# awslabs/dgl-ke

Hardware: NVIDIA H100
Metric: edges/sec TransE_l2 d=400 neg=200 at 1/2/4/8 H100 vs ref CPU; HBM GB/s %peak (higher is better)
Workload: dtype f32

## Files before the change

### dgl-ke_b200/csrc/kge_fused.cu

```cuda
#include <cuda.h>
#include <cstdio>
#include <cstdlib>
#include "kge_common.cuh"
#include "kge_tc.cuh"

namespace kge {

using namespace tc;

namespace {

constexpr int kTileM = 128;
constexpr int kThreadsF = 384;
constexpr int kProducerWarp = 8;
constexpr int kMaxS1 = 4, kMaxS2 = 8;
constexpr int kMaxPf = 8;
constexpr uint32_t kRingBytes = 192 * 1024;
constexpr int kWc = 128;
constexpr float kLog2e = 1.4426950408889634f;
constexpr float kLn2 = 0.6931471805599453f;

struct FusedArgs {
  int model, adversarial;
  float gamma, Tl2e, inv2B, uni;
  float reg_coef;
  int reg_norm;
  int C, Rx, Ry, D;
  int N1;
  int nblkD;
  int nS1, nS2;
  uint32_t stage1Bytes, stage2Bytes;
  float *VhiT, *VloT;
  float* colpart;
  int ncolpart;
  const float* x2;
  const float* y2;
  const float* pos;
  const float* wt;
  const float* wbar;
  float *gpos, *rowsum, *pl, *nl;
  float* dumpS;
// ... 53 lines not shown
  };
  for (long long k = 0; k < n && k < S; ++k) load(k);
  const int L = g.pf_lag < S - 1 ? g.pf_lag : (S > 2 ? S - 2 : 1);
  for (long long k = 0; k < n; ++k) {
    const int s = (int)(k % S);
    mbar_wait(&pf_full[w][s], (uint32_t)((k / S) & 1));
    const long long v = vrow(k);
    float* dst = v < nU ? g.pf_nc + v * (long long)g.D : g.pf_bn + (v - nU) * (long long)g.D;
    const long long kr = k - L + S;
    const bool reload = k >= L && kr < n;
    if (reload && kr >= base + 32) { base += 32; ids_lo = ids_hi; ids_hi = fetch_ids(base + 32); }
    if (elect_one()) {
      bulk_s2g(dst, slots + (size_t)s * g.pf_row_bytes, g.pf_row_bytes);
      bulk_commit();
      if (reload) { if (L == 3) bulk_wait_read<3>(); else if (L == 2) bulk_wait_read<2>(); else bulk_wait_read<1>(); }
    }
    __syncwarp();
    if (reload) load(kr);
  }
  if (elect_one()) bulk_wait_all();
  __syncwarp();
}

template <int NV>
__global__ void __launch_bounds__(kThreadsF, 1)
k_fused_pos(const __grid_constant__ CUtensorMap mXh, const __grid_constant__ CUtensorMap mXl,
            const __grid_constant__ CUtensorMap mYh1, const __grid_constant__ CUtensorMap mYl1,
            const __grid_constant__ CUtensorMap mYh2, const __grid_constant__ CUtensorMap mYl2, FusedArgs g) {
  extern __shared__ __align__(1024) uint8_t smem_raw[];
  __shared__ __align__(8) uint64_t full1[kMaxS1], empty1[kMaxS1], full2[kMaxS2], empty2[kMaxS2];
  __shared__ __align__(8) uint64_t pf_full[2][kMaxPf];
  __shared__ __align__(16) float colA[NV];
  __shared__ __align__(16) float cpart[8][NV];

  const int warp = threadIdx.x >> 5, lane = threadIdx.x & 31;
  uint8_t* ring = (uint8_t*)(((uintptr_t)smem_raw + 1023) & ~(uintptr_t)1023);

  const int mtiles = (g.Rx + kTileM - 1) / kTileM;
  const int ntiles = g.C * mtiles;
  const int nkb1 = (g.D + 31) >> 5;
  const int nkb2 = (g.Ry + 31) >> 5;
  const int nchunks = (g.D + kWc - 1) / kWc;
  constexpr uint32_t yBytes1 = (uint32_t)NV * 128u;
  constexpr uint32_t yBytes2 = (uint32_t)kWc * 128u;
  const bool l2 = g.model == KGE_TRANSE_L2;

  if (threadIdx.x == 0) {
    for (int s = 0; s < kMaxS1; ++s) { mbar_init(&full1[s], 1); mbar_init(&empty1[s], 8); }
    for (int s = 0; s < kMaxS2; ++s) { mbar_init(&full2[s], 1); mbar_init(&empty2[s], 8); }
    for (int s = 0; s < kMaxPf; ++s) { mbar_init(&pf_full[0][s], 1); mbar_init(&pf_full[1][s], 1); }
    asm volatile("fence.mbarrier_init.release.cluster;" ::: "memory");
  }
  if (warp == kProducerWarp && lane == 0) {
    tma_prefetch_desc(&mXh); tma_prefetch_desc(&mXl); tma_prefetch_desc(&mYh1);
    tma_prefetch_desc(&mYl1); tma_prefetch_desc(&mYh2); tma_prefetch_desc(&mYl2);
  }
  __syncthreads();

  if (warp >= 8) {
  asm volatile("setmaxnreg.dec.sync.aligned.u32 56;");
  if (warp == kProducerWarp) {
    uint32_t n1 = 0, n2 = 0;
    for (int tile = blockIdx.x; tile < ntiles; tile += gridDim.x) {
      const int c = tile / mtiles, m0 = (tile % mtiles) * kTileM;
      for (uint32_t k = (n2 > (uint32_t)g.nS2 ? n2 - g.nS2 : 0); k < n2; ++k) mbar_wait(&empty2[k % g.nS2], (k / g.nS2) & 1);
      for (int kb = 0; kb < nkb1; ++kb, ++n1) {
        const uint32_t s = n1 % g.nS1;
        mbar_wait(&empty1[s], ((n1 / g.nS1) & 1) ^ 1);
        uint8_t* st = ring + (size_t)s * g.stage1Bytes;
        const int yx = (c * g.nblkD + kb) * g.Rx + m0;
        const int yy = (c * g.nblkD + kb) * g.Ry;
        if (elect_one()) {
          mbar_expect_tx(&full1[s], 2u * 16384u + 2u * yBytes1);
          tma_load_2d(st, &mXh, &full1[s], 0, yx);
          tma_load_2d(st + 16384, &mXl, &full1[s], 0, yx);
          tma_load_2d(st + 32768, &mYh1, &full1[s], 0, yy);
          tma_load_2d(st + 32768 + yBytes1, &mYl1, &full1[s], 0, yy);
        }
        __syncwarp();
      }
      for (uint32_t k = (n1 > (uint32_t)g.nS1 ? n1 - g.nS1 : 0); k < n1; ++k) mbar_wait(&empty1[k % g.nS1], (k / g.nS1) & 1);
      for (int ch = 0; ch < nchunks; ++ch) {
        for (int kb = 0; kb < nkb2; ++kb, ++n2) {
          const uint32_t s = n2 % g.nS2;
          mbar_wait(&empty2[s], ((n2 / g.nS2) & 1) ^ 1);
          uint8_t* st = ring + (size_t)s * g.stage2Bytes;
          const int yy = (c * nkb2 + kb) * g.D + ch * kWc;
          if (elect_one()) {
            mbar_expect_tx(&full2[s], 2u * yBytes2);
            tma_load_2d(st, &mYh2, &full2[s], 0, yy);
            tma_load_2d(st + yBytes2, &mYl2, &full2[s], 0, yy);
          }
          __syncwarp();
        }
      }
    }
  } else if (warp >= 10 && g.pf_slots > 0) {
    prefetch_rows(g, ring, pf_full, warp - 10, lane);
  }
  } else {
    asm volatile("setmaxnreg.inc.sync.aligned.u32 224;");
    const int wg = warp >> 2, q = lane & 3;
    const int et = threadIdx.x;
    const int rloc = wg * 64 + (warp & 3) * 16 + (lane >> 2);
    uint32_t n1 = 0, n2 = 0;
    float acc[NV / 2];
    for (int tile = blockIdx.x; tile < ntiles; tile += gridDim.x) {
      const int c = tile / mtiles, m0 = (tile % mtiles) * kTileM;
      epi_bar();
      for (int y = et; y < NV; y += 256) {
        const bool ok = y < g.Ry;
        colA[y] = (l2 && ok) ? g.y2[(long long)c * g.Ry + y] : 0.f;
      }
      epi_bar();
#pragma unroll
      for (int i = 0; i < NV / 2; ++i) acc[i] = 0.f;
      for (int kb = 0; kb < nkb1; ++kb, ++n1) {
        const uint32_t s = n1 % g.nS1;
        mbar_wait(&full1[s], (n1 / g.nS1) & 1);
        const uint32_t st = smem_u32(ring + (size_t)s * g.stage1Bytes);
        const uint64_t dXh = make_desc(st + wg * 8192u), dXl = make_desc(st + 16384u + wg * 8192u);
        const uint64_t dYh = make_desc(st + 32768u), dYl = make_desc(st + 32768u + yBytes1);
        const int kleft = g.D - kb * 32;
        const int ksteps = kleft >= 32 ? 4 : (kleft >> 3);
        wgmma_fence();
        for (int ks = 0; ks < ksteps; ++ks) {
          const uint64_t o = (uint64_t)(ks * 2);
          wgmma_ss<NV>(acc, dXh + o, dYh + o, 1u);
          wgmma_ss<NV>(acc, dXh + o, dYl + o, 1u);
          wgmma_ss<NV>(acc, dXl + o, dYh + o, 1u);
        }
        wgmma_commit();
        if (kb > 0) {
          wgmma_wait<1>();
          if (lane == 0) mbar_arrive(&empty1[(n1 - 1) % g.nS1]);
        }
      }
      wgmma_wait<0>();
      if (lane == 0) mbar_arrive(&empty1[(n1 - 1) % g.nS1]);
      reg_fence(acc);

      float rscal[2];
#pragma unroll
      for (int h = 0; h < 2; ++h) {
        const int m = m0 + rloc + 8 * h;
        const bool row_ok = m < g.Rx;
        const long long gx = (long long)c * g.Rx + (row_ok ? m : 0);
        const float x2v = (l2 && row_ok) ? g.x2[gx] : 0.f;
        const float w_i = (g.wt && row_ok) ? g.wt[gx] : 1.f;
        const float kw = w_i * g.inv2B;
        float mxl = -INFINITY;
        if (g.adversarial || g.dumpS) {
#pragma unroll
          for (int j = 0; j < NV / 8; ++j) {
            float sv[2];
// ... 37 lines not shown
            const float u = 1.f + t;
            const float r1 = rcpa(u);
            const float sig = (s >= 0.f) ? r1 : t * r1;
            const float sp = fmaf(kLn2, lg2a(u), fmaxf(s, 0.f));
            const bool ok = row_ok && (col < g.Ry);
            const float coef = ok ? pe * sig * kw * rinv : 0.f;
            if (ok) { nls = fmaf(pe, sp, nls); den += pe; }
            rs += coef;
            acc[4 * j + 2 * h + e] = coef;
          }
        }
        den += __shfl_xor_sync(0xffffffffu, den, 1); den += __shfl_xor_sync(0xffffffffu, den, 2);
        nls += __shfl_xor_sync(0xffffffffu, nls, 1); nls += __shfl_xor_sync(0xffffffffu, nls, 2);
        rs += __shfl_xor_sync(0xffffffffu, rs, 1); rs += __shfl_xor_sync(0xffffffffu, rs, 2);
        const float rscale = g.adversarial ? (row_ok ? 1.f / den : 0.f) : g.uni;
        rscal[h] = rscale;
        if (g.dumpV && row_ok) {
#pragma unroll
          for (int j = 0; j < NV / 8; ++j)
            if (8 * j + 2 * q < g.Ry)
              *reinterpret_cast<float2*>(g.dumpV + gx * g.Ry + 8 * j + 2 * q) =
                  make_float2(acc[4 * j + 2 * h] * rscale, acc[4 * j + 2 * h + 1] * rscale);
        }
        {
          float* vh = g.VhiT + slabT_off(c, g.Rx, g.Ry, m, 0);
          float* vl = g.VloT + slabT_off(c, g.Rx, g.Ry, m, 0);
#pragma unroll
          for (int j = 0; j < NV / 8; ++j) {
#pragma unroll
            for (int e = 0; e < 2; ++e) {
              const int col = 8 * j + 2 * q + e;
              const float v = acc[4 * j + 2 * h + e] * rscale;
              if (row_ok && col < g.Ry) {
                float hi, lo;
                split_tf32(v, hi, lo);
                vh[col * 32] = hi; vl[col * 32] = lo;
              }
              if (l2) {
                float s = v;
                s += __shfl_xor_sync(0xffffffffu, s, 4);
                s += __shfl_xor_sync(0xffffffffu, s, 8);
                s += __shfl_xor_sync(0xffffffffu, s, 16);
                if (lane < 4) cpart[warp][col] = h ? cpart[warp][col] + s : s;
              }
            }
          }
        }
        if (q == 0 && row_ok) {
          const float ps = g.pos[gx];
          const float wb = g.wt ? *g.wbar : 1.f;
          g.pl[gx] = softplusf(-ps);
          g.nl[gx] = nls * rscale * w_i;
          g.gpos[gx] = -sigmoidf(-ps) * wb * g.inv2B;
          if (l2) g.rowsum[gx] = rs * rscale;
        }
      }
      if (l2) {
        epi_bar();
        float* dst = g.colpart + (long long)(tile % mtiles) * g.C * g.Ry + (long long)c * g.Ry;
        for (int y = et; y < g.Ry; y += 256) {
          float s = cpart[0][y];
#pragma unroll
          for (int w = 1; w < 8; ++w) s += cpart[w][y];
          dst[y] = s;
        }
      }
      {
        const int srcLo = (lane & ~3) | (q >> 1), srcHi = srcLo + 2;
        const bool odd = q & 1;
#pragma unroll
        for (int j = 0; j < NV / 8; ++j) {
          float o[4];
#pragma unroll
          for (int h = 0; h < 2; ++h) {
            const float v0 = acc[4 * j + 2 * h], v1 = acc[4 * j + 2 * h + 1];
            const float a0 = __shfl_sync(0xffffffffu, v0, srcLo), a1 = __shfl_sync(0xffffffffu, v1, srcLo);
            const float b0 = __shfl_sync(0xffffffffu, v0, srcHi), b1 = __shfl_sync(0xffffffffu, v1, srcHi);
            o[h] = odd ? a1 : a0;
            o[2 + h] = odd ? b1 : b0;
          }
          acc[4 * j + 0] = o[0]; acc[4 * j + 1] = o[1]; acc[4 * j + 2] = o[2]; acc[4 * j + 3] = o[3];
        }
      }

      for (int ch = 0; ch < nchunks; ++ch) {
        const int d0 = ch * kWc;
        float acc2[kWc / 2];
#pragma unroll
        for (int i = 0; i < kWc / 2; ++i) acc2[i] = 0.f;
#pragma unroll
        for (int kb = 0; kb < (NV + 31) / 32; ++kb) {
          if (kb >= nkb2) break;
          const uint32_t s = n2 % g.nS2;
          mbar_wait(&full2[s], (n2 / g.nS2) & 1);
          const uint32_t st = smem_u32(ring + (size_t)s * g.stage2Bytes);
          const uint64_t dYh = make_desc(st), dYl = make_desc(st + yBytes2);
          const int kleft = g.Ry - kb * 32;
          const int ksteps = kleft >= 32 ? 4 : (kleft >> 3);
          uint32_t ah[2][4] = {}, al[2][4] = {};
#pragma unroll
          for (int ks = 0; ks < 4; ++ks) {
            const int j = kb * 4 + ks;
            if (j < NV / 8 && ks < ksteps) {
              if (ks >= 2) wgmma_wait<1>();
#pragma unroll
              for (int r = 0; r < 4; ++r) {
                float hi, lo;
                split_tf32(acc[4 * j + r], hi, lo);
                ah[ks & 1][r] = __float_as_uint(hi); al[ks & 1][r] = __float_as_uint(lo);
              }
              wgmma_fence();
              const uint64_t o = (uint64_t)(ks * 2);
              wgmma_rs<kWc>(acc2, ah[ks & 1], dYh + o, 1u);
              wgmma_rs<kWc>(acc2, ah[ks & 1], dYl + o, 1u);
              wgmma_rs<kWc>(acc2, al[ks & 1], dYh + o, 1u);
              wgmma_commit();
              if (ks >= 1) { reg_fence(ah[(ks - 1) & 1]); reg_fence(al[(ks - 1) & 1]); }
            }
          }
          wgmma_wait<0>();
          reg_fence(ah[0]); reg_fence(ah[1]); reg_fence(al[0]); reg_fence(al[1]);
          if (lane == 0) mbar_arrive(&empty2[s]);
          ++n2;
        }
        reg_fence(acc2);
#pragma unroll
        for (int h = 0; h < 2; ++h) {
          const int m = m0 + rloc + 8 * h;
          if (m >= g.Rx) continue;
          float* orow = g.out + ((long long)c * g.Rx + m) * (long long)g.D;
#pragma unroll
          for (int j = 0; j < kWc / 8; ++j) {
            const int k = d0 + 8 * j + 2 * q;
            if (k >= g.D) continue;
            *reinterpret_cast<float2*>(orow + k) = make_float2(acc2[4 * j + 2 * h] * rscal[h], acc2[4 * j + 2 * h + 1] * rscal[h]);
          }
        }
      }
    }
  }
}

template <int NW, int KS>
__device__ __forceinline__ void neg_kblock(float (&acc)[NW / 2], uint64_t dVh, uint64_t dVl, uint64_t dAh, uint64_t dAl) {
  wgmma_fence();
#pragma unroll
  for (int ks = 0; ks < KS; ++ks) {
    const uint64_t o = (uint64_t)(ks * 2);
    wgmma_ss<NW>(acc, dVh + o, dAh + o, 1u);
    wgmma_ss<NW>(acc, dVh + o, dAl + o, 1u);
    wgmma_ss<NW>(acc, dVl + o, dAh + o, 1u);
  }
  wgmma_commit();
}

constexpr int kNegEpiLoads = 16;

template <int NW, bool FLAT>
__global__ void __launch_bounds__(kThreadsF, 1)
k_fused_neg(const __grid_constant__ CUtensorMap mVh, const __grid_constant__ CUtensorMap mVl,
            const __grid_constant__ CUtensorMap mAh, const __grid_constant__ CUtensorMap mAl, FusedArgs g) {
  extern __shared__ __align__(1024) uint8_t smem_raw[];
  __shared__ __align__(8) uint64_t full[kMaxS1], empty[kMaxS1];
  __shared__ __align__(8) uint64_t pf_full[2][kMaxPf];

  const int warp = threadIdx.x >> 5, lane = threadIdx.x & 31;
  uint8_t* ring = (uint8_t*)(((uintptr_t)smem_raw + 1023) & ~(uintptr_t)1023);

  const int mtiles = (g.Rx + kTileM - 1) / kTileM;
  const int ntiles = g.C * mtiles;
  const int nkb = (g.Ry + 31) >> 5;
  const int nch = (g.D + NW - 1) / NW;
  constexpr uint32_t aBytes = (uint32_t)kTileM * 128u;
  constexpr uint32_t bBytes = (uint32_t)NW * 128u;
  const bool l2 = g.model == KGE_TRANSE_L2;

  if (threadIdx.x == 0) {
// ... 84 lines not shown
          if (FLAT) {
            bh[jj] = __ldg(reinterpret_cast<const float2*>(brow[h] + k));
          } else {
            const long long so = boff[h] + (k >> 5) * blk + (k & 31);
            bh[jj] = __ldg(reinterpret_cast<const float2*>(g.Xhi + so));
            bl[jj] = __ldg(reinterpret_cast<const float2*>(g.Xlo + so));
          }
        }
      };
      float gsq[2] = {0.f, 0.f};
      for (int ch = 0; ch < nch; ++ch) {
        const int d0 = ch * NW;
        float acc[NW / 2];
#pragma unroll
        for (int i = 0; i < NW / 2; ++i) acc[i] = 0.f;
        for (int kb = 0; kb < nkb; ++kb, ++n) {
          const uint32_t s = n % g.nS1;
          mbar_wait(&full[s], (n / g.nS1) & 1);
          const uint32_t st = smem_u32(ring + (size_t)s * g.stage1Bytes);
          const uint64_t dVh = make_desc(st + wg * 8192u), dVl = make_desc(st + aBytes + wg * 8192u);
          const uint64_t dAh = make_desc(st + 2 * aBytes), dAl = make_desc(st + 2 * aBytes + bBytes);
          const int kleft = g.Ry - kb * 32;
          const int ksteps = kleft >= 32 ? 4 : (kleft >> 3);
          switch (ksteps) {
            case 4: neg_kblock<NW, 4>(acc, dVh, dVl, dAh, dAl); break;
            case 3: neg_kblock<NW, 3>(acc, dVh, dVl, dAh, dAl); break;
            case 2: neg_kblock<NW, 2>(acc, dVh, dVl, dAh, dAl); break;
            default: neg_kblock<NW, 1>(acc, dVh, dVl, dAh, dAl); break;
          }
          if (kb > 0) {
            wgmma_wait<1>();
            if (lane == 0) mbar_arrive(&empty[(n - 1) % g.nS1]);
          }
        }
        if (early) load_b(0, d0, 0);
        wgmma_wait<0>();
        if (lane == 0) mbar_arrive(&empty[(n - 1) % g.nS1]);
        reg_fence(acc);
#pragma unroll
        for (int h = 0; h < 2; ++h) {
          if (!rok[h]) continue;
          float* orow = g.out + ((long long)c * g.Rx + m0 + rloc + 8 * h) * (long long)g.D;
#pragma unroll
          for (int j0 = 0; j0 < NJ; j0 += NB) {
            if (!early || h > 0 || j0 > 0) load_b(h, d0, j0);
#pragma unroll
            for (int jj = 0; jj < NB; ++jj) {
              const int j = j0 + jj;
              const int k = d0 + 8 * j + 2 * q;
              if (j >= NJ || k >= g.D) continue;
              float o0 = acc[4 * j + 2 * h], o1 = acc[4 * j + 2 * h + 1];
              const float2 b = FLAT ? bh[jj] : make_float2(bh[jj].x + bl[jj].x, bh[jj].y + bl[jj].y);
// ... 5 lines not shown
            }
          }
        }
      }
#pragma unroll
      for (int h = 0; h < 2; ++h) {
        float v = gsq[h];
        v += __shfl_xor_sync(0xffffffffu, v, 1);
        v += __shfl_xor_sync(0xffffffffu, v, 2);
        const int m = m0 + rloc + 8 * h;
        if (q == 0 && m < g.Rx) g.gsn[(long long)c * g.Rx + m] = v / (float)g.D;
      }
    }
  }
}

}

bool fused_supported(const StepParams& p) {
  return umma_supported(p) && !p.hinge && !p.pairwise && !p.neg_deg && p.Cs <= 240 && p.Ns <= 240;
}

namespace {
struct Geometry { int Rx, Ry, N1, nS1, nS2, pf_slots; uint32_t stage1Bytes, stage2Bytes, pf_off; bool ok; };

int neg_chunk_width(int D, bool want_prefetch) {
  static const int widths[] = {64, 128, 200, 256};
  int best = 0;
  long long best_rows = 0;
  for (int w : widths) {
    if (w == 256 && want_prefetch) continue;
    const long long rows = (long long)((D + w - 1) / w) * (kTileM + w);
    if (!best || rows < best_rows) { best = w; best_rows = rows; }
  }
  return best;
}

Geometry geometry(const StepParams& p, int mode, bool want_prefetch) {
  Geometry q{};
  const uint32_t row = (uint32_t)p.D * 4u;
  if (mode == 1) {
    q.Rx = p.Ns; q.Ry = p.Cs;
    q.N1 = neg_chunk_width(p.D, want_prefetch);
    q.stage1Bytes = 2u * kTileM * 128u + 2u * (uint32_t)q.N1 * 128u;
    q.nS1 = (int)(kRingBytes / q.stage1Bytes); if (q.nS1 > kMaxS1) q.nS1 = kMaxS1;
    q.ok = q.nS1 >= 2;
    if (q.ok && want_prefetch) {
      int nS = q.nS1;
      while (nS > 2 && kRingBytes - (uint32_t)nS * q.stage1Bytes < 2u * kMaxPf * row) --nS;
      const uint32_t used = (uint32_t)nS * q.stage1Bytes;
      int slots = (int)((kRingBytes - used) / (2u * row));
      if (slots > kMaxPf) slots = kMaxPf;
      if (slots >= 2) { q.pf_slots = slots; q.nS1 = nS; q.pf_off = used; }
    }
    return q;
  }
  q.Rx = p.Cs; q.Ry = p.Ns;
  q.N1 = q.Ry <= 64 ? 64 : (q.Ry <= 128 ? 128 : (q.Ry <= 208 ? 208 : 256));
  q.stage1Bytes = 2u * 16384u + 2u * (uint32_t)q.N1 * 128u;
  q.stage2Bytes = 2u * (uint32_t)kWc * 128u;
  q.nS1 = (int)(kRingBytes / q.stage1Bytes); if (q.nS1 > kMaxS1) q.nS1 = kMaxS1;
  q.nS2 = (int)(kRingBytes / q.stage2Bytes); if (q.nS2 > kMaxS2) q.nS2 = kMaxS2;
  q.ok = q.nS1 >= 2 && q.nS2 >= 2;
  if (q.ok && want_prefetch) {
    int nS1 = q.nS1, nS2 = q.nS2;
    uint32_t want = 2u * kMaxPf * row;
    while (nS1 > 2 && kRingBytes - (uint32_t)nS1 * q.stage1Bytes < want) --nS1;
    uint32_t used = (uint32_t)nS1 * q.stage1Bytes;
    if (want > kRingBytes - used) want = kRingBytes - used;
    while (nS2 > 4 && kRingBytes - (uint32_t)nS2 * q.stage2Bytes < want) --nS2;
    if ((uint32_t)nS2 * q.stage2Bytes > used) used = (uint32_t)nS2 * q.stage2Bytes;
    int slots = (int)((kRingBytes - used) / (2u * row));
    if (slots > kMaxPf) slots = kMaxPf;
    if (slots >= 2) { q.pf_slots = slots; q.nS1 = nS1; q.nS2 = nS2; q.pf_off = used; }
  }
  return q;
}

int launch_error() {
  const cudaError_t e = cudaGetLastError();
  return e == cudaSuccess ? KGE_OK : fail(KGE_ERR_CUDA, "k_fused launch: %s", cudaGetErrorString(e));
}
template <int NV>
int launch_pos(const LaunchCtx& c, int grid, size_t smem, const CUtensorMap* m, const FusedArgs& g) {
  if (int rc = smem_optin((const void*)k_fused_pos<NV>, smem)) return rc;
  KGE_LAUNCH_NAMED(c, "k_fused<P: S=A.Bn^T, loss, GA=V.Bn>", (k_fused_pos<NV>), grid, kThreadsF, smem,
                   m[0], m[1], m[2], m[3], m[4], m[5], g);
  return launch_error();
}
template <int NW, bool FLAT>
int launch_neg_src(const LaunchCtx& c, int grid, size_t smem, const CUtensorMap* m, const FusedArgs& g) {
  if (int rc = smem_optin((const void*)k_fused_neg<NW, FLAT>, smem)) return rc;
  KGE_LAUNCH_NAMED(c, "k_fused<N: G_neg=V^T.A, mean sq>", (k_fused_neg<NW, FLAT>), grid, kThreadsF, smem, m[0], m[1], m[2], m[3], g);
  return launch_error();
}
template <int NW>
int launch_neg(const LaunchCtx& c, int grid, size_t smem, const CUtensorMap* m, const FusedArgs& g) {
  return (g.xraw || g.xids) ? launch_neg_src<NW, true>(c, grid, smem, m, g) : launch_neg_src<NW, false>(c, grid, smem, m, g);
}
int launch_width(const LaunchCtx& c, bool P, int grid, size_t smem, const CUtensorMap* m, const FusedArgs& g) {
  switch (g.N1) {
    case 64: return P ? launch_pos<64>(c, grid, smem, m, g) : launch_neg<64>(c, grid, smem, m, g);
    case 128: return P ? launch_pos<128>(c, grid, smem, m, g) : launch_neg<128>(c, grid, smem, m, g);
    case 200: return launch_neg<200>(c, grid, smem, m, g);
    case 208: return launch_pos<208>(c, grid, smem, m, g);
    default: return P ? launch_pos<256>(c, grid, smem, m, g) : launch_neg<256>(c, grid, smem, m, g);
  }
}
}

int fused_prefetch_slots(const StepParams& p, int mode) { return geometry(p, mode, true).pf_slots; }

int fused_launch(const LaunchCtx& c, const StepParams& p, const StepWs& w, int mode, const float* wt, float* dumpS,
                 float* dumpV, const TableView* ent, const long long* neg_ids, const FusedPrefetch* pf) {
  FusedArgs g{};
  g.model = p.model; g.adversarial = p.adversarial;
  g.gamma = p.gamma; g.Tl2e = p.adv_temperature * kLog2e; g.inv2B = 0.5f / (float)p.B; g.uni = 1.f / (float)p.Ns;
  g.reg_coef = p.reg_coef; g.reg_norm = p.reg_norm;
  g.C = p.C; g.D = p.D; g.nblkD = slab_blocks(p.D);
  const bool P = mode == 0;
  const Geometry q = geometry(p, mode, pf != nullptr && ent != nullptr);
  if (!q.ok) return fail(KGE_ERR_UNSUPPORTED, "fused kernel: shape does not fit (N1=%d)", q.N1);
  g.Rx = q.Rx; g.Ry = q.Ry; g.N1 = q.N1; g.nS1 = q.nS1; g.nS2 = q.nS2;
  g.stage1Bytes = q.stage1Bytes; g.stage2Bytes = q.stage2Bytes;
  if (pf && ent && q.pf_slots >= 2) {
    static const int lag_env = getenv("KGE_B200_PF_LAG") ? atoi(getenv("KGE_B200_PF_LAG")) : 1;
    g.pf_lag = lag_env < 1 ? 1 : (lag_env > 3 ? 3 : lag_env);
    g.pf_slots = q.pf_slots; g.pf_off = q.pf_off; g.pf_row_bytes = (uint32_t)p.D * 4u; g.pf_parity = mode;
    g.pf_node_ids = pf->node_ids; g.pf_nU_dev = pf->nU_dev; g.pf_nU = pf->nU; g.pf_nNeg = pf->nNeg;
    g.pf_neg_ids = pf->neg_ids; g.pf_nc = pf->nc; g.pf_bn = pf->bn;
    g.xtab = *ent;
  }
  g.VhiT = w.VhiT; g.VloT = w.VloT; g.colpart = w.colpart; g.ncolpart = (p.Cs + kTileM - 1) / kTileM;
  g.dumpV = dumpV;
  const size_t smem = kRingBytes + 1024;
  const int mtiles = (g.Rx + kTileM - 1) / kTileM;
  int grid = p.C * mtiles;
  if (grid > c.num_sms) grid = c.num_sms;
  CUtensorMap m[6];
  if (P) {
    g.x2 = w.a2; g.y2 = w.b2;
    g.pos = w.pos; g.wt = wt; g.wbar = w.wbar;
    g.gpos = w.gpos; g.rowsum = w.rowsum; g.pl = w.pl; g.nl = w.nl;
    g.dumpS = dumpS;
    g.out = w.GA;
    const long long rowsX = (long long)p.C * p.Cs * g.nblkD, rowsY = (long long)p.C * p.Ns * g.nblkD;
    const long long rowsYT = (long long)p.C * slab_blocks(p.Ns) * p.D;
    if (tc_make_map(&m[0], w.Ahi, rowsX, 32, kTileM) || tc_make_map(&m[1], w.Alo, rowsX, 32, kTileM) ||
        tc_make_map(&m[2], w.Bhi, rowsY, 32, g.N1) || tc_make_map(&m[3], w.Blo, rowsY, 32, g.N1) ||
        tc_make_map(&m[4], w.BhiT, rowsYT, 32, kWc) || tc_make_map(&m[5], w.BloT, rowsYT, 32, kWc))
      return KGE_ERR_CUDA;
    return launch_width(c, true, grid, smem, m, g);
  }
  g.Xhi = w.Bhi; g.Xlo = w.Blo;
  if (ent && ent->n_shards == 1 && neg_ids) { g.xids = neg_ids; g.xtab = *ent; }
  if (w.BnRaw) g.xraw = w.BnRaw;
  g.gsn = w.gsn;
  g.out = w.Bn;
  const long long rowsV = (long long)p.C * slab_blocks(p.Cs) * p.Ns, rowsA = (long long)p.C * slab_blocks(p.Cs) * p.D;
  if (tc_make_map(&m[0], w.VhiT, rowsV, 32, kTileM) || tc_make_map(&m[1], w.VloT, rowsV, 32, kTileM) ||
      tc_make_map(&m[2], w.AhiT, rowsA, 32, g.N1) || tc_make_map(&m[3], w.AloT, rowsA, 32, g.N1))
    return KGE_ERR_CUDA;
  return launch_width(c, false, grid, smem, m, g);
}

}
```

### dgl-ke_b200/csrc/kge_tc.cuh

```cuda
#pragma once
#include <cuda.h>
#include <cuda_runtime.h>
#include <stdint.h>

namespace kge {
namespace tc {

__device__ __forceinline__ uint32_t smem_u32(const void* p) { return (uint32_t)__cvta_generic_to_shared(p); }

__device__ __forceinline__ bool elect_one() {
  uint32_t pred = 0;
  asm volatile(
      "{\n\t.reg .pred P1;\n\t"
      "elect.sync _|P1, 0xFFFFFFFF;\n\t"
      "selp.b32 %0, 1, 0, P1;\n\t}"
      : "=r"(pred));
  return pred != 0;
}

__device__ __forceinline__ void mbar_init(uint64_t* bar, uint32_t count) {
  asm volatile("mbarrier.init.shared::cta.b64 [%0], %1;" ::"r"(smem_u32(bar)), "r"(count));
}
__device__ __forceinline__ void mbar_expect_tx(uint64_t* bar, uint32_t bytes) {
  asm volatile("mbarrier.arrive.expect_tx.shared::cta.b64 _, [%0], %1;" ::"r"(smem_u32(bar)), "r"(bytes) : "memory");
// ... 66 lines not shown
}
template <>
__device__ __forceinline__ void wgmma_ss<200>(float (&d)[100], uint64_t adesc, uint64_t bdesc, uint32_t accumulate) {
  asm volatile("{\n\t.reg .pred p;\n\tsetp.ne.b32 p, %102, 0;\n\t"
               "wgmma.mma_async.sync.aligned.m64n200k8.f32.tf32.tf32 {%0,%1,%2,%3,%4,%5,%6,%7,%8,%9,%10,%11,%12,%13,%14,%15,%16,%17,%18,%19,%20,%21,%22,%23,%24,%25,%26,%27,%28,%29,%30,%31,%32,%33,%34,%35,%36,%37,%38,%39,%40,%41,%42,%43,%44,%45,%46,%47,%48,%49,%50,%51,%52,%53,%54,%55,%56,%57,%58,%59,%60,%61,%62,%63,%64,%65,%66,%67,%68,%69,%70,%71,%72,%73,%74,%75,%76,%77,%78,%79,%80,%81,%82,%83,%84,%85,%86,%87,%88,%89,%90,%91,%92,%93,%94,%95,%96,%97,%98,%99}, %100, %101, p, 1, 1;\n\t}"
               : KGE_D32(0), KGE_D32(32), KGE_D32(64), KGE_D4(96)
               : "l"(adesc), "l"(bdesc), "r"(accumulate));
}
template <>
__device__ __forceinline__ void wgmma_ss<208>(float (&d)[104], uint64_t adesc, uint64_t bdesc, uint32_t accumulate) {
  asm volatile("{\n\t.reg .pred p;\n\tsetp.ne.b32 p, %106, 0;\n\t"
               "wgmma.mma_async.sync.aligned.m64n208k8.f32.tf32.tf32 {%0,%1,%2,%3,%4,%5,%6,%7,%8,%9,%10,%11,%12,%13,%14,%15,%16,%17,%18,%19,%20,%21,%22,%23,%24,%25,%26,%27,%28,%29,%30,%31,%32,%33,%34,%35,%36,%37,%38,%39,%40,%41,%42,%43,%44,%45,%46,%47,%48,%49,%50,%51,%52,%53,%54,%55,%56,%57,%58,%59,%60,%61,%62,%63,%64,%65,%66,%67,%68,%69,%70,%71,%72,%73,%74,%75,%76,%77,%78,%79,%80,%81,%82,%83,%84,%85,%86,%87,%88,%89,%90,%91,%92,%93,%94,%95,%96,%97,%98,%99,%100,%101,%102,%103}, %104, %105, p, 1, 1;\n\t}"
               : KGE_D32(0), KGE_D32(32), KGE_D32(64), KGE_D4(96), KGE_D4(100)
               : "l"(adesc), "l"(bdesc), "r"(accumulate));
}
template <>
__device__ __forceinline__ void wgmma_ss<256>(float (&d)[128], uint64_t adesc, uint64_t bdesc, uint32_t accumulate) {
  asm volatile("{\n\t.reg .pred p;\n\tsetp.ne.b32 p, %130, 0;\n\t"
               "wgmma.mma_async.sync.aligned.m64n256k8.f32.tf32.tf32 {%0,%1,%2,%3,%4,%5,%6,%7,%8,%9,%10,%11,%12,%13,%14,%15,%16,%17,%18,%19,%20,%21,%22,%23,%24,%25,%26,%27,%28,%29,%30,%31,%32,%33,%34,%35,%36,%37,%38,%39,%40,%41,%42,%43,%44,%45,%46,%47,%48,%49,%50,%51,%52,%53,%54,%55,%56,%57,%58,%59,%60,%61,%62,%63,%64,%65,%66,%67,%68,%69,%70,%71,%72,%73,%74,%75,%76,%77,%78,%79,%80,%81,%82,%83,%84,%85,%86,%87,%88,%89,%90,%91,%92,%93,%94,%95,%96,%97,%98,%99,%100,%101,%102,%103,%104,%105,%106,%107,%108,%109,%110,%111,%112,%113,%114,%115,%116,%117,%118,%119,%120,%121,%122,%123,%124,%125,%126,%127}, %128, %129, p, 1, 1;\n\t}"
               : KGE_D32(0), KGE_D32(32), KGE_D32(64), KGE_D32(96)
               : "l"(adesc), "l"(bdesc), "r"(accumulate));
}
template <>
__device__ __forceinline__ void wgmma_rs<128>(float (&d)[64], const uint32_t (&a)[4], uint64_t bdesc, uint32_t accumulate) {
  asm volatile("{\n\t.reg .pred p;\n\tsetp.ne.b32 p, %69, 0;\n\t"
               "wgmma.mma_async.sync.aligned.m64n128k8.f32.tf32.tf32 {%0,%1,%2,%3,%4,%5,%6,%7,%8,%9,%10,%11,%12,%13,%14,%15,%16,%17,%18,%19,%20,%21,%22,%23,%24,%25,%26,%27,%28,%29,%30,%31,%32,%33,%34,%35,%36,%37,%38,%39,%40,%41,%42,%43,%44,%45,%46,%47,%48,%49,%50,%51,%52,%53,%54,%55,%56,%57,%58,%59,%60,%61,%62,%63}, {%64,%65,%66,%67}, %68, p, 1, 1;\n\t}"
               : KGE_D32(0), KGE_D32(32)
               : "r"(a[0]), "r"(a[1]), "r"(a[2]), "r"(a[3]), "l"(bdesc), "r"(accumulate));
}
#undef KGE_D4
#undef KGE_D16
#undef KGE_D32

__device__ __forceinline__ uint64_t make_desc(uint32_t saddr) {
  uint64_t d = 0;
  d |= (uint64_t)((saddr >> 4) & 0x3FFF);
  d |= (uint64_t)1 << 16;
  d |= (uint64_t)(1024 >> 4) << 32;
  d |= (uint64_t)1 << 62;
  return d;
}

__device__ __forceinline__ float ex2a(float x) { float y; asm("ex2.approx.ftz.f32 %0, %1;" : "=f"(y) : "f"(x)); return y; }
__device__ __forceinline__ float lg2a(float x) { float y; asm("lg2.approx.ftz.f32 %0, %1;" : "=f"(y) : "f"(x)); return y; }
__device__ __forceinline__ float rcpa(float x) { float y; asm("rcp.approx.ftz.f32 %0, %1;" : "=f"(y) : "f"(x)); return y; }
__device__ __forceinline__ float rsqrta(float x) { float y; asm("rsqrt.approx.ftz.f32 %0, %1;" : "=f"(y) : "f"(x)); return y; }
// ... 8 lines not shown
```

Measured before the change: 29.57 million.

## Pick GEMM2 chunk width per D and stream V stores inside first chunk

The second GEMM (gradient = V·B^T) in the positive fused kernel used a fixed 128-column chunk, which pads D=400 up to 512 columns. The chunk width is now chosen from 64, 80 or 128 to minimise padded columns, and any remainder is covered with power-of-two tail chunks (64/32/16/8) loaded by narrow TMA maps. The V hi/lo split-and-store that used to happen in the epilogue is now interleaved into the first GEMM2 chunk, and the k-step loop is restructured with per-kstep stage release. This adds more template instantiations and extra register pressure from keeping V stores in the GEMM2 loop.

```diff
diff --git a/dgl-ke_b200/csrc/kge_fused.cu b/dgl-ke_b200/csrc/kge_fused.cu
--- a/dgl-ke_b200/csrc/kge_fused.cu
+++ b/dgl-ke_b200/csrc/kge_fused.cu
@@ -16,7 +16,6 @@
 constexpr int kMaxS1 = 4, kMaxS2 = 8;
 constexpr int kMaxPf = 8;
 constexpr uint32_t kRingBytes = 192 * 1024;
-constexpr int kWc = 128;
 constexpr float kLog2e = 1.4426950408889634f;
 constexpr float kLn2 = 0.6931471805599453f;
 
@@ -116,11 +115,116 @@
   __syncwarp();
 }
 
+template <int N, int KS>
+__device__ __forceinline__ void kblock_ss(float (&acc)[N / 2], uint64_t dAh, uint64_t dAl, uint64_t dBh, uint64_t dBl) {
+  wgmma_fence();
+#pragma unroll
+  for (int ks = 0; ks < KS; ++ks) {
+    const uint64_t o = (uint64_t)(ks * 2);
+    wgmma_ss<N>(acc, dAh + o, dBh + o, 1u);
+    wgmma_ss<N>(acc, dAh + o, dBl + o, 1u);
+    wgmma_ss<N>(acc, dAl + o, dBh + o, 1u);
+  }
+  wgmma_commit();
+}
+template <int N>
+__device__ __forceinline__ void kblock_ss(float (&acc)[N / 2], int ksteps, uint64_t dAh, uint64_t dAl, uint64_t dBh,
+                                          uint64_t dBl) {
+  switch (ksteps) {
+    case 4: kblock_ss<N, 4>(acc, dAh, dAl, dBh, dBl); break;
+    case 3: kblock_ss<N, 3>(acc, dAh, dAl, dBh, dBl); break;
+    case 2: kblock_ss<N, 2>(acc, dAh, dAl, dBh, dBl); break;
+    default: kblock_ss<N, 1>(acc, dAh, dAl, dBh, dBl); break;
+  }
+}
+
+struct VOut { float *hi, *lo; bool rok0, rok1; };
+
 template <int NV>
+__device__ __forceinline__ void store_v_kstep(const FusedArgs& g, const float (&v)[NV / 2], int j, const VOut& vo,
+                                              const float (&rscal)[2]) {
+  const int q = threadIdx.x & 3;
+#pragma unroll
+  for (int r = 0; r < 4; ++r) {
+    const int h = r & 1, cj = 8 * j + 4 * (r >> 1);
+    if ((h ? vo.rok1 : vo.rok0) && cj + q < g.Ry) {
+      float hi, lo;
+      split_tf32(v[4 * j + r] * rscal[h], hi, lo);
+      vo.hi[cj * 32 + 8 * h] = hi; vo.lo[cj * 32 + 8 * h] = lo;
+    }
+  }
+}
+
+template <int NV, int CW, bool SV = false>
+__device__ __forceinline__ void gemm2_chunk(const FusedArgs& g, const float (&v)[NV / 2], const uint8_t* ring,
+                                            uint64_t* full2, uint64_t* empty2, uint32_t& n2, int c, int m0, int rloc,
+                                            int d0, const float (&rscal)[2], const VOut& vo) {
+  const int lane = threadIdx.x & 31, q = lane & 3;
+  const int nks = g.Ry >> 3, nkb = (g.Ry + 31) >> 5;
+  float acc2[CW / 2];
+#pragma unroll
+  for (int i = 0; i < CW / 2; ++i) acc2[i] = 0.f;
+  uint32_t ah[2][4], al[2][4];
+  uint32_t rel = n2;
+  uint64_t dYh = 0, dYl = 0;
+#pragma unroll
+  for (int j = 0; j < NV / 8; ++j) {
+    const int ks = j & 3;
+    const bool live = j < nks;
+    if (ks == 0 && live) {
+      const uint32_t n = n2 + j / 4, s = n % g.nS2;
+      mbar_wait(&full2[s], (n / g.nS2) & 1);
+      const uint32_t st = smem_u32(ring + (size_t)s * g.stage2Bytes);
+      dYh = make_desc(st); dYl = make_desc(st + CW * 128u);
+    }
+    if (j >= 2) {
+      wgmma_wait<1>();
+      if (ks == 1 && j - 2 < nks) {
+        if (lane == 0) mbar_arrive(&empty2[rel % g.nS2]);
+        ++rel;
+      }
+    }
+#pragma unroll
+    for (int r = 0; r < 4; ++r) {
+      float hi, lo;
+      split_tf32(v[4 * j + r], hi, lo);
+      ah[j & 1][r] = __float_as_uint(hi); al[j & 1][r] = __float_as_uint(lo);
+    }
+    wgmma_fence();
+    const uint64_t o = live ? (uint64_t)(ks * 2) : 0;
+    wgmma_rs<CW>(acc2, ah[j & 1], dYh + o, 1u);
+    wgmma_rs<CW>(acc2, ah[j & 1], dYl + o, 1u);
+    wgmma_rs<CW>(acc2, al[j & 1], dYh + o, 1u);
+    wgmma_commit();
+    if (j >= 1) { reg_fence(ah[(j - 1) & 1]); reg_fence(al[(j - 1) & 1]); }
+    if (SV && live) store_v_kstep<NV>(g, v, j, vo, rscal);
+  }
+  wgmma_wait<0>();
+  reg_fence(ah[0]); reg_fence(ah[1]); reg_fence(al[0]); reg_fence(al[1]);
+  for (; rel < n2 + nkb; ++rel)
+    if (lane == 0) mbar_arrive(&empty2[rel % g.nS2]);
+  n2 += nkb;
+  reg_fence(acc2);
+#pragma unroll
+  for (int h = 0; h < 2; ++h) {
+    const int m = m0 + rloc + 8 * h;
+    if (m >= g.Rx) continue;
+    float* orow = g.out + ((long long)c * g.Rx + m) * (long long)g.D;
+#pragma unroll
+    for (int j = 0; j < CW / 8; ++j) {
+      const int k = d0 + 8 * j + 2 * q;
+      if (k >= g.D) continue;
+      *reinterpret_cast<float2*>(orow + k) = make_float2(acc2[4 * j + 2 * h] * rscal[h], acc2[4 * j + 2 * h + 1] * rscal[h]);
+    }
+  }
+}
+
+template <int NV, int W>
 __global__ void __launch_bounds__(kThreadsF, 1)
 k_fused_pos(const __grid_constant__ CUtensorMap mXh, const __grid_constant__ CUtensorMap mXl,
             const __grid_constant__ CUtensorMap mYh1, const __grid_constant__ CUtensorMap mYl1,
-            const __grid_constant__ CUtensorMap mYh2, const __grid_constant__ CUtensorMap mYl2, FusedArgs g) {
+            const __grid_constant__ CUtensorMap mYh2, const __grid_constant__ CUtensorMap mYl2,
+            const __grid_constant__ CUtensorMap mYh8, const __grid_constant__ CUtensorMap mYl8, FusedArgs g) {
   extern __shared__ __align__(1024) uint8_t smem_raw[];
   __shared__ __align__(8) uint64_t full1[kMaxS1], empty1[kMaxS1], full2[kMaxS2], empty2[kMaxS2];
   __shared__ __align__(8) uint64_t pf_full[2][kMaxPf];
@@ -134,9 +238,9 @@
   const int ntiles = g.C * mtiles;
   const int nkb1 = (g.D + 31) >> 5;
   const int nkb2 = (g.Ry + 31) >> 5;
-  const int nchunks = (g.D + kWc - 1) / kWc;
+  const int nfull = ((g.D + 7) & ~7) / W;
+  const int rest = ((g.D + 7) & ~7) - nfull * W;
   constexpr uint32_t yBytes1 = (uint32_t)NV * 128u;
-  constexpr uint32_t yBytes2 = (uint32_t)kWc * 128u;
   const bool l2 = g.model == KGE_TRANSE_L2;
 
   if (threadIdx.x == 0) {
@@ -148,6 +252,7 @@
   if (warp == kProducerWarp && lane == 0) {
     tma_prefetch_desc(&mXh); tma_prefetch_desc(&mXl); tma_prefetch_desc(&mYh1);
     tma_prefetch_desc(&mYl1); tma_prefetch_desc(&mYh2); tma_prefetch_desc(&mYl2);
+    if (rest) { tma_prefetch_desc(&mYh8); tma_prefetch_desc(&mYl8); }
   }
   __syncthreads();
 
@@ -174,20 +279,32 @@
         __syncwarp();
       }
       for (uint32_t k = (n1 > (uint32_t)g.nS1 ? n1 - g.nS1 : 0); k < n1; ++k) mbar_wait(&empty1[k % g.nS1], (k / g.nS1) & 1);
-      for (int ch = 0; ch < nchunks; ++ch) {
+      auto fill2 = [&](int d0, int cw) {
+        const uint32_t yBytes2 = (uint32_t)cw * 128u;
         for (int kb = 0; kb < nkb2; ++kb, ++n2) {
           const uint32_t s = n2 % g.nS2;
           mbar_wait(&empty2[s], ((n2 / g.nS2) & 1) ^ 1);
           uint8_t* st = ring + (size_t)s * g.stage2Bytes;
-          const int yy = (c * nkb2 + kb) * g.D + ch * kWc;
+          const int yy = (c * nkb2 + kb) * g.D + d0;
           if (elect_one()) {
             mbar_expect_tx(&full2[s], 2u * yBytes2);
-            tma_load_2d(st, &mYh2, &full2[s], 0, yy);
-            tma_load_2d(st + yBytes2, &mYl2, &full2[s], 0, yy);
+            if (cw == W) {
+              tma_load_2d(st, &mYh2, &full2[s], 0, yy);
+              tma_load_2d(st + yBytes2, &mYl2, &full2[s], 0, yy);
+            } else {
+              for (int r = 0; r < cw; r += 8) {
+                tma_load_2d(st + r * 128, &mYh8, &full2[s], 0, yy + r);
+                tma_load_2d(st + yBytes2 + r * 128, &mYl8, &full2[s], 0, yy + r);
+              }
+            }
           }
           __syncwarp();
         }
-      }
+      };
+      int d0 = 0;
+      for (int ch = 0; ch < nfull; ++ch, d0 += W) fill2(d0, W);
+      for (int p = 64; p >= 8; p >>= 1)
+        if (rest & p) { fill2(d0, p); d0 += p; }
     }
   } else if (warp >= 10 && g.pf_slots > 0) {
     prefetch_rows(g, ring, pf_full, warp - 10, lane);
@@ -216,15 +333,7 @@
         const uint64_t dXh = make_desc(st + wg * 8192u), dXl = make_desc(st + 16384u + wg * 8192u);
         const uint64_t dYh = make_desc(st + 32768u), dYl = make_desc(st + 32768u + yBytes1);
         const int kleft = g.D - kb * 32;
-        const int ksteps = kleft >= 32 ? 4 : (kleft >> 3);
-        wgmma_fence();
-        for (int ks = 0; ks < ksteps; ++ks) {
-          const uint64_t o = (uint64_t)(ks * 2);
-          wgmma_ss<NV>(acc, dXh + o, dYh + o, 1u);
-          wgmma_ss<NV>(acc, dXh + o, dYl + o, 1u);
-          wgmma_ss<NV>(acc, dXl + o, dYh + o, 1u);
-        }
-        wgmma_commit();
+        kblock_ss<NV>(acc, kleft >= 32 ? 4 : (kleft >> 3), dXh, dXl, dYh, dYl);
         if (kb > 0) {
           wgmma_wait<1>();
           if (lane == 0) mbar_arrive(&empty1[(n1 - 1) % g.nS1]);
@@ -308,27 +417,17 @@
               *reinterpret_cast<float2*>(g.dumpV + gx * g.Ry + 8 * j + 2 * q) =
                   make_float2(acc[4 * j + 2 * h] * rscale, acc[4 * j + 2 * h + 1] * rscale);
         }
-        {
-          float* vh = g.VhiT + slabT_off(c, g.Rx, g.Ry, m, 0);
-          float* vl = g.VloT + slabT_off(c, g.Rx, g.Ry, m, 0);
+        if (l2) {
 #pragma unroll
           for (int j = 0; j < NV / 8; ++j) {
 #pragma unroll
             for (int e = 0; e < 2; ++e) {
               const int col = 8 * j + 2 * q + e;
-              const float v = acc[4 * j + 2 * h + e] * rscale;
-              if (row_ok && col < g.Ry) {
-                float hi, lo;
-                split_tf32(v, hi, lo);
-                vh[col * 32] = hi; vl[col * 32] = lo;
-              }
-              if (l2) {
-                float s = v;
-                s += __shfl_xor_sync(0xffffffffu, s, 4);
-                s += __shfl_xor_sync(0xffffffffu, s, 8);
-                s += __shfl_xor_sync(0xffffffffu, s, 16);
-                if (lane < 4) cpart[warp][col] = h ? cpart[warp][col] + s : s;
-              }
+              float s = acc[4 * j + 2 * h + e] * rscale;
+              s += __shfl_xor_sync(0xffffffffu, s, 4);
+              s += __shfl_xor_sync(0xffffffffu, s, 8);
+              s += __shfl_xor_sync(0xffffffffu, s, 16);
+              if (lane < 4) cpart[warp][col] = h ? cpart[warp][col] + s : s;
             }
           }
         }
@@ -369,76 +468,27 @@
         }
       }
 
-      for (int ch = 0; ch < nchunks; ++ch) {
-        const int d0 = ch * kWc;
-        float acc2[kWc / 2];
-#pragma unroll
-        for (int i = 0; i < kWc / 2; ++i) acc2[i] = 0.f;
-#pragma unroll
-        for (int kb = 0; kb < (NV + 31) / 32; ++kb) {
-          if (kb >= nkb2) break;
-          const uint32_t s = n2 % g.nS2;
-          mbar_wait(&full2[s], (n2 / g.nS2) & 1);
-          const uint32_t st = smem_u32(ring + (size_t)s * g.stage2Bytes);
-          const uint64_t dYh = make_desc(st), dYl = make_desc(st + yBytes2);
-          const int kleft = g.Ry - kb * 32;
-          const int ksteps = kleft >= 32 ? 4 : (kleft >> 3);
-          uint32_t ah[2][4] = {}, al[2][4] = {};
-#pragma unroll
-          for (int ks = 0; ks < 4; ++ks) {
-            const int j = kb * 4 + ks;
-            if (j < NV / 8 && ks < ksteps) {
-              if (ks >= 2) wgmma_wait<1>();
-#pragma unroll
-              for (int r = 0; r < 4; ++r) {
-                float hi, lo;
-                split_tf32(acc[4 * j + r], hi, lo);
-                ah[ks & 1][r] = __float_as_uint(hi); al[ks & 1][r] = __float_as_uint(lo);
-              }
-              wgmma_fence();
-              const uint64_t o = (uint64_t)(ks * 2);
-              wgmma_rs<kWc>(acc2, ah[ks & 1], dYh + o, 1u);
-              wgmma_rs<kWc>(acc2, ah[ks & 1], dYl + o, 1u);
-              wgmma_rs<kWc>(acc2, al[ks & 1], dYh + o, 1u);
-              wgmma_commit();
-              if (ks >= 1) { reg_fence(ah[(ks - 1) & 1]); reg_fence(al[(ks - 1) & 1]); }
-            }
-          }
-          wgmma_wait<0>();
-          reg_fence(ah[0]); reg_fence(ah[1]); reg_fence(al[0]); reg_fence(al[1]);
-          if (lane == 0) mbar_arrive(&empty2[s]);
-          ++n2;
-        }
-        reg_fence(acc2);
-#pragma unroll
-        for (int h = 0; h < 2; ++h) {
-          const int m = m0 + rloc + 8 * h;
-          if (m >= g.Rx) continue;
-          float* orow = g.out + ((long long)c * g.Rx + m) * (long long)g.D;
-#pragma unroll
-          for (int j = 0; j < kWc / 8; ++j) {
-            const int k = d0 + 8 * j + 2 * q;
-            if (k >= g.D) continue;
-            *reinterpret_cast<float2*>(orow + k) = make_float2(acc2[4 * j + 2 * h] * rscal[h], acc2[4 * j + 2 * h + 1] * rscal[h]);
-          }
-        }
-      }
-    }
-  }
-}
-
-template <int NW, int KS>
-__device__ __forceinline__ void neg_kblock(float (&acc)[NW / 2], uint64_t dVh, uint64_t dVl, uint64_t dAh, uint64_t dAl) {
-  wgmma_fence();
-#pragma unroll
-  for (int ks = 0; ks < KS; ++ks) {
-    const uint64_t o = (uint64_t)(ks * 2);
-    wgmma_ss<NW>(acc, dVh + o, dAh + o, 1u);
-    wgmma_ss<NW>(acc, dVh + o, dAl + o, 1u);
-    wgmma_ss<NW>(acc, dVl + o, dAh + o, 1u);
-  }
-  wgmma_commit();
-}
+      const VOut vo{g.VhiT + slabT_off(c, g.Rx, g.Ry, m0 + rloc, q), g.VloT + slabT_off(c, g.Rx, g.Ry, m0 + rloc, q),
+                    m0 + rloc < g.Rx, m0 + rloc + 8 < g.Rx};
+      int d0 = 0, ch = 0;
+      if (NV < 256 && nfull) {
+        gemm2_chunk<NV, W, NV < 256>(g, acc, ring, full2, empty2, n2, c, m0, rloc, d0, rscal, vo);
+        d0 += W; ch = 1;
+      } else {
+#pragma unroll
+        for (int j = 0; j < NV / 8; ++j) store_v_kstep<NV>(g, acc, j, vo, rscal);
+      }
+      for (; ch < nfull; ++ch, d0 += W) gemm2_chunk<NV, W>(g, acc, ring, full2, empty2, n2, c, m0, rloc, d0, rscal, vo);
+      if constexpr (W > 64) {
+        if (rest & 64) { gemm2_chunk<NV, 64>(g, acc, ring, full2, empty2, n2, c, m0, rloc, d0, rscal, vo); d0 += 64; }
+      }
+      if (rest & 32) { gemm2_chunk<NV, 32>(g, acc, ring, full2, empty2, n2, c, m0, rloc, d0, rscal, vo); d0 += 32; }
+      if (rest & 16) { gemm2_chunk<NV, 16>(g, acc, ring, full2, empty2, n2, c, m0, rloc, d0, rscal, vo); d0 += 16; }
+      if (rest & 8) gemm2_chunk<NV, 8>(g, acc, ring, full2, empty2, n2, c, m0, rloc, d0, rscal, vo);
+    }
+  }
+}
+
 
 constexpr int kNegEpiLoads = 16;
 
@@ -569,12 +619,7 @@
           const uint64_t dAh = make_desc(st + 2 * aBytes), dAl = make_desc(st + 2 * aBytes + bBytes);
           const int kleft = g.Ry - kb * 32;
           const int ksteps = kleft >= 32 ? 4 : (kleft >> 3);
-          switch (ksteps) {
-            case 4: neg_kblock<NW, 4>(acc, dVh, dVl, dAh, dAl); break;
-            case 3: neg_kblock<NW, 3>(acc, dVh, dVl, dAh, dAl); break;
-            case 2: neg_kblock<NW, 2>(acc, dVh, dVl, dAh, dAl); break;
-            default: neg_kblock<NW, 1>(acc, dVh, dVl, dAh, dAl); break;
-          }
+          kblock_ss<NW>(acc, ksteps, dVh, dVl, dAh, dAl);
           if (kb > 0) {
             wgmma_wait<1>();
             if (lane == 0) mbar_arrive(&empty[(n - 1) % g.nS1]);
@@ -626,7 +671,7 @@
 }
 
 namespace {
-struct Geometry { int Rx, Ry, N1, nS1, nS2, pf_slots; uint32_t stage1Bytes, stage2Bytes, pf_off; bool ok; };
+struct Geometry { int Rx, Ry, N1, W2, nS1, nS2, pf_slots; uint32_t stage1Bytes, stage2Bytes, pf_off; bool ok; };
 
 int neg_chunk_width(int D, bool want_prefetch) {
   static const int widths[] = {64, 128, 200, 256};
@@ -636,6 +681,19 @@
     if (w == 256 && want_prefetch) continue;
     const long long rows = (long long)((D + w - 1) / w) * (kTileM + w);
     if (!best || rows < best_rows) { best = w; best_rows = rows; }
+  }
+  return best;
+}
+
+constexpr bool pos_width_built(int NV, int W) { return (W == 64 || W == 80 || W == 128) && (NV < 256 || W == 64); }
+
+int pos_chunk_width(int D, int NV) {
+  static const int widths[] = {64, 80, 128};
+  int best = 0, best_cols = 0, best_n = 0;
+  for (int w : widths) {
+    if (!pos_width_built(NV, w)) continue;
+    const int n = (D + w - 1) / w, cols = n * w;
+    if (!best || cols < best_cols || (cols == best_cols && n < best_n)) { best = w; best_cols = cols; best_n = n; }
   }
   return best;
 }
@@ -662,7 +720,8 @@
   q.Rx = p.Cs; q.Ry = p.Ns;
   q.N1 = q.Ry <= 64 ? 64 : (q.Ry <= 128 ? 128 : (q.Ry <= 208 ? 208 : 256));
   q.stage1Bytes = 2u * 16384u + 2u * (uint32_t)q.N1 * 128u;
-  q.stage2Bytes = 2u * (uint32_t)kWc * 128u;
+  q.W2 = pos_chunk_width(p.D, q.N1);
+  q.stage2Bytes = 2u * (uint32_t)q.W2 * 128u;
   q.nS1 = (int)(kRingBytes / q.stage1Bytes); if (q.nS1 > kMaxS1) q.nS1 = kMaxS1;
   q.nS2 = (int)(kRingBytes / q.stage2Bytes); if (q.nS2 > kMaxS2) q.nS2 = kMaxS2;
   q.ok = q.nS1 >= 2 && q.nS2 >= 2;
@@ -685,12 +744,25 @@
   const cudaError_t e = cudaGetLastError();
   return e == cudaSuccess ? KGE_OK : fail(KGE_ERR_CUDA, "k_fused launch: %s", cudaGetErrorString(e));
 }
+template <int NV, int W>
+int launch_pos_w(const LaunchCtx& c, int grid, size_t smem, const CUtensorMap* m, const FusedArgs& g) {
+  if constexpr (!pos_width_built(NV, W)) {
+    return fail(KGE_ERR_UNSUPPORTED, "k_fused<P>: no variant for GEMM1 width %d and chunk width %d", NV, W);
+  } else {
+    if (int rc = smem_optin((const void*)k_fused_pos<NV, W>, smem)) return rc;
+    KGE_LAUNCH_NAMED(c, "k_fused<P: S=A.Bn^T, loss, GA=V.Bn>", (k_fused_pos<NV, W>), grid, kThreadsF, smem,
+                     m[0], m[1], m[2], m[3], m[4], m[5], m[6], m[7], g);
+    return launch_error();
+  }
+}
 template <int NV>
-int launch_pos(const LaunchCtx& c, int grid, size_t smem, const CUtensorMap* m, const FusedArgs& g) {
-  if (int rc = smem_optin((const void*)k_fused_pos<NV>, smem)) return rc;
-  KGE_LAUNCH_NAMED(c, "k_fused<P: S=A.Bn^T, loss, GA=V.Bn>", (k_fused_pos<NV>), grid, kThreadsF, smem,
-                   m[0], m[1], m[2], m[3], m[4], m[5], g);
-  return launch_error();
+int launch_pos(const LaunchCtx& c, int grid, size_t smem, const CUtensorMap* m, const FusedArgs& g, int W) {
+  switch (W) {
+    case 64: return launch_pos_w<NV, 64>(c, grid, smem, m, g);
+    case 80: return launch_pos_w<NV, 80>(c, grid, smem, m, g);
+    case 128: return launch_pos_w<NV, 128>(c, grid, smem, m, g);
+    default: return fail(KGE_ERR_UNSUPPORTED, "k_fused<P>: no GEMM2 chunk width for GEMM1 width %d", NV);
+  }
 }
 template <int NW, bool FLAT>
 int launch_neg_src(const LaunchCtx& c, int grid, size_t smem, const CUtensorMap* m, const FusedArgs& g) {
@@ -702,13 +774,13 @@
 int launch_neg(const LaunchCtx& c, int grid, size_t smem, const CUtensorMap* m, const FusedArgs& g) {
   return (g.xraw || g.xids) ? launch_neg_src<NW, true>(c, grid, smem, m, g) : launch_neg_src<NW, false>(c, grid, smem, m, g);
 }
-int launch_width(const LaunchCtx& c, bool P, int grid, size_t smem, const CUtensorMap* m, const FusedArgs& g) {
+int launch_width(const LaunchCtx& c, bool P, int grid, size_t smem, const CUtensorMap* m, const FusedArgs& g, int W) {
   switch (g.N1) {
-    case 64: return P ? launch_pos<64>(c, grid, smem, m, g) : launch_neg<64>(c, grid, smem, m, g);
-    case 128: return P ? launch_pos<128>(c, grid, smem, m, g) : launch_neg<128>(c, grid, smem, m, g);
+    case 64: return P ? launch_pos<64>(c, grid, smem, m, g, W) : launch_neg<64>(c, grid, smem, m, g);
+    case 128: return P ? launch_pos<128>(c, grid, smem, m, g, W) : launch_neg<128>(c, grid, smem, m, g);
     case 200: return launch_neg<200>(c, grid, smem, m, g);
-    case 208: return launch_pos<208>(c, grid, smem, m, g);
-    default: return P ? launch_pos<256>(c, grid, smem, m, g) : launch_neg<256>(c, grid, smem, m, g);
+    case 208: return launch_pos<208>(c, grid, smem, m, g, W);
+    default: return P ? launch_pos<256>(c, grid, smem, m, g, W) : launch_neg<256>(c, grid, smem, m, g);
   }
 }
 }
@@ -741,7 +813,7 @@
   const int mtiles = (g.Rx + kTileM - 1) / kTileM;
   int grid = p.C * mtiles;
   if (grid > c.num_sms) grid = c.num_sms;
-  CUtensorMap m[6];
+  CUtensorMap m[8];
   if (P) {
     g.x2 = w.a2; g.y2 = w.b2;
     g.pos = w.pos; g.wt = wt; g.wbar = w.wbar;
@@ -752,9 +824,11 @@
     const long long rowsYT = (long long)p.C * slab_blocks(p.Ns) * p.D;
     if (tc_make_map(&m[0], w.Ahi, rowsX, 32, kTileM) || tc_make_map(&m[1], w.Alo, rowsX, 32, kTileM) ||
         tc_make_map(&m[2], w.Bhi, rowsY, 32, g.N1) || tc_make_map(&m[3], w.Blo, rowsY, 32, g.N1) ||
-        tc_make_map(&m[4], w.BhiT, rowsYT, 32, kWc) || tc_make_map(&m[5], w.BloT, rowsYT, 32, kWc))
+        tc_make_map(&m[4], w.BhiT, rowsYT, 32, q.W2) || tc_make_map(&m[5], w.BloT, rowsYT, 32, q.W2))
       return KGE_ERR_CUDA;
-    return launch_width(c, true, grid, smem, m, g);
+    if (((p.D + 7) & ~7) % q.W2 == 0) { m[6] = m[4]; m[7] = m[5]; }
+    else if (tc_make_map(&m[6], w.BhiT, rowsYT, 32, 8) || tc_make_map(&m[7], w.BloT, rowsYT, 32, 8)) return KGE_ERR_CUDA;
+    return launch_width(c, true, grid, smem, m, g, q.W2);
   }
   g.Xhi = w.Bhi; g.Xlo = w.Blo;
   if (ent && ent->n_shards == 1 && neg_ids) { g.xids = neg_ids; g.xtab = *ent; }
@@ -765,7 +839,7 @@
   if (tc_make_map(&m[0], w.VhiT, rowsV, 32, kTileM) || tc_make_map(&m[1], w.VloT, rowsV, 32, kTileM) ||
       tc_make_map(&m[2], w.AhiT, rowsA, 32, g.N1) || tc_make_map(&m[3], w.AloT, rowsA, 32, g.N1))
     return KGE_ERR_CUDA;
-  return launch_width(c, false, grid, smem, m, g);
-}
-
-}
+  return launch_width(c, false, grid, smem, m, g, 0);
+}
+
+}
diff --git a/dgl-ke_b200/csrc/kge_tc.cuh b/dgl-ke_b200/csrc/kge_tc.cuh
--- a/dgl-ke_b200/csrc/kge_tc.cuh
+++ b/dgl-ke_b200/csrc/kge_tc.cuh
@@ -112,6 +112,41 @@
                : "l"(adesc), "l"(bdesc), "r"(accumulate));
 }
 template <>
+__device__ __forceinline__ void wgmma_rs<8>(float (&d)[4], const uint32_t (&a)[4], uint64_t bdesc, uint32_t accumulate) {
+  asm volatile("{\n\t.reg .pred p;\n\tsetp.ne.b32 p, %9, 0;\n\t"
+               "wgmma.mma_async.sync.aligned.m64n8k8.f32.tf32.tf32 {%0,%1,%2,%3}, {%4,%5,%6,%7}, %8, p, 1, 1;\n\t}"
+               : KGE_D4(0)
+               : "r"(a[0]), "r"(a[1]), "r"(a[2]), "r"(a[3]), "l"(bdesc), "r"(accumulate));
+}
+template <>
+__device__ __forceinline__ void wgmma_rs<16>(float (&d)[8], const uint32_t (&a)[4], uint64_t bdesc, uint32_t accumulate) {
+  asm volatile("{\n\t.reg .pred p;\n\tsetp.ne.b32 p, %13, 0;\n\t"
+               "wgmma.mma_async.sync.aligned.m64n16k8.f32.tf32.tf32 {%0,%1,%2,%3,%4,%5,%6,%7}, {%8,%9,%10,%11}, %12, p, 1, 1;\n\t}"
+               : KGE_D4(0), KGE_D4(4)
+               : "r"(a[0]), "r"(a[1]), "r"(a[2]), "r"(a[3]), "l"(bdesc), "r"(accumulate));
+}
+template <>
+__device__ __forceinline__ void wgmma_rs<32>(float (&d)[16], const uint32_t (&a)[4], uint64_t bdesc, uint32_t accumulate) {
+  asm volatile("{\n\t.reg .pred p;\n\tsetp.ne.b32 p, %21, 0;\n\t"
+               "wgmma.mma_async.sync.aligned.m64n32k8.f32.tf32.tf32 {%0,%1,%2,%3,%4,%5,%6,%7,%8,%9,%10,%11,%12,%13,%14,%15}, {%16,%17,%18,%19}, %20, p, 1, 1;\n\t}"
+               : KGE_D16(0)
+               : "r"(a[0]), "r"(a[1]), "r"(a[2]), "r"(a[3]), "l"(bdesc), "r"(accumulate));
+}
+template <>
+__device__ __forceinline__ void wgmma_rs<64>(float (&d)[32], const uint32_t (&a)[4], uint64_t bdesc, uint32_t accumulate) {
+  asm volatile("{\n\t.reg .pred p;\n\tsetp.ne.b32 p, %37, 0;\n\t"
+               "wgmma.mma_async.sync.aligned.m64n64k8.f32.tf32.tf32 {%0,%1,%2,%3,%4,%5,%6,%7,%8,%9,%10,%11,%12,%13,%14,%15,%16,%17,%18,%19,%20,%21,%22,%23,%24,%25,%26,%27,%28,%29,%30,%31}, {%32,%33,%34,%35}, %36, p, 1, 1;\n\t}"
+               : KGE_D32(0)
+               : "r"(a[0]), "r"(a[1]), "r"(a[2]), "r"(a[3]), "l"(bdesc), "r"(accumulate));
+}
+template <>
+__device__ __forceinline__ void wgmma_rs<80>(float (&d)[40], const uint32_t (&a)[4], uint64_t bdesc, uint32_t accumulate) {
+  asm volatile("{\n\t.reg .pred p;\n\tsetp.ne.b32 p, %45, 0;\n\t"
+               "wgmma.mma_async.sync.aligned.m64n80k8.f32.tf32.tf32 {%0,%1,%2,%3,%4,%5,%6,%7,%8,%9,%10,%11,%12,%13,%14,%15,%16,%17,%18,%19,%20,%21,%22,%23,%24,%25,%26,%27,%28,%29,%30,%31,%32,%33,%34,%35,%36,%37,%38,%39}, {%40,%41,%42,%43}, %44, p, 1, 1;\n\t}"
+               : KGE_D32(0), KGE_D4(32), KGE_D4(36)
+               : "r"(a[0]), "r"(a[1]), "r"(a[2]), "r"(a[3]), "l"(bdesc), "r"(accumulate));
+}
+template <>
 __device__ __forceinline__ void wgmma_rs<128>(float (&d)[64], const uint32_t (&a)[4], uint64_t bdesc, uint32_t accumulate) {
   asm volatile("{\n\t.reg .pred p;\n\tsetp.ne.b32 p, %69, 0;\n\t"
                "wgmma.mma_async.sync.aligned.m64n128k8.f32.tf32.tf32 {%0,%1,%2,%3,%4,%5,%6,%7,%8,%9,%10,%11,%12,%13,%14,%15,%16,%17,%18,%19,%20,%21,%22,%23,%24,%25,%26,%27,%28,%29,%30,%31,%32,%33,%34,%35,%36,%37,%38,%39,%40,%41,%42,%43,%44,%45,%46,%47,%48,%49,%50,%51,%52,%53,%54,%55,%56,%57,%58,%59,%60,%61,%62,%63}, {%64,%65,%66,%67}, %68, p, 1, 1;\n\t}"
```

New measurement: 29.61 million (median of 6 runs). No clear change (+0.1%).
